# pnnl/nmrfit

Hardware: AMD Instinct MI355X
Metric: objective evals/sec (swarm x grid x peaks) (higher is better)
Workload: dtype f64

## Files before the change

### nmrfit_amd/csrc/objective_pair.h

```cpp
#pragma once
#include "objective_chunk.h"
#include "objective_finish.h"
#include "objective_launch.h"
#include "objective_lds.h"
#include "objective_prologue.h"
#include "swarm_prologue.h"

#include <type_traits>

namespace nmrfit {
namespace {

struct PairSide {
    PeakLor *lor;
    PeakFast *lorf;
    double2 *grec;
    PeakWin *win;
    double2 *seeds;
    double *shr;
    double *state;
    double *wsums;
    double base;
    bool rec_all;
};

template <bool FAST, bool FULL>
__device__ __forceinline__ void pair_model(const PairSide &s, const int P, const int lane, const double2 mm,
                                           const double (&wv)[kPointsPerLane], double (&acc)[kPointsPerLane])
{
    const double base = s.base;
    int k = 0;
    {
        const int kend0 = (P < kWave) ? P : kWave;
        if (kGroupSize <= kend0) {
            if constexpr (FAST)
                lorentz_group_fast<kGroupSize, true>(s.lorf, wv, acc, base);
            else
                lorentz_group<kGroupSize, true>(s.lor, wv, acc, base);
            k = kGroupSize;
        } else if (kend0 > 0) {
            if constexpr (FAST)
                lorentz_tail_fast<true>(kend0, s.lorf, wv, acc, base);
            else
                lorentz_tail<kGroupSize, true>(kend0, s.lor, wv, acc, base);
            k = kend0;
        } else {
#pragma unroll
            for (int q = 0; q < kPointsPerLane; ++q) acc[q] = base;
        }
    }
    for (int kb = 0; kb < P; kb += kWave) {
        const int kend = (P < kb + kWave) ? P : kb + kWave;
        bool h = false;
        if (kb + lane < P) {
            const PeakWin wn = s.win[kb + lane];
            h = (mm.y >= (double)wn.lo) && (mm.x <= (double)wn.hi);
        }
        unsigned long long hits = __ballot(h);
        if (kb != 0) k = kb;
        if constexpr (FAST) {
            for (; k + kGroupSize <= kend; k += kGroupSize) lorentz_group_fast<kGroupSize>(s.lorf + k, wv, acc);
            if (k < kend) lorentz_tail_fast(kend - k, s.lorf + k, wv, acc);
        } else {
            for (; k + kGroupSize <= kend; k += kGroupSize) lorentz_group<kGroupSize>(s.lor + k, wv, acc);
            if (k < kend) lorentz_tail<kGroupSize>(kend - k, s.lor + k, wv, acc);
        }
        if (kend - kb < kWave) hits &= (1ull << (kend - kb)) - 1ull;
        const bool rec = FULL && s.rec_all;
        for (unsigned long long m = rec ? hits : 0ull; m; m &= m - 1) {
            const int k1 = kb + __builtin_ctzll(m);
            gauss_add_rec(s.lor + k1, s.grec + k1, wv, acc);
        }
        for (unsigned long long m = rec ? 0ull : hits; m; m &= m - 1) gauss_add<true>(s.lor + kb + __builtin_ctzll(m), wv, acc);
    }
}

struct PairState {
    double zr, zi, bs;
};
__device__ __forceinline__ PairState pair_state(const PairSide &s, const int lane, const bool first, const int bidx)
{
    PairState st;
    if (first) {
        const double2 e = s.seeds[bidx];
        const double lr = s.shr[2 + lane], li = s.shr[2 + kWave + lane];
        st.zr = __builtin_fma(e.x, lr, -(e.y * li));
        st.zi = __builtin_fma(e.x, li, e.y * lr);
    } else {
        st.zr = s.state[lane];
        st.zi = s.state[kWave + lane];
    }
    st.bs = s.state[2 * kWave + lane];
    return st;
}

__device__ __forceinline__ void pair_epilogue(const PairSide &s, const int lane, const PairState &st, const bool last, const int slot,
                                              const double (&acc)[kPointsPerLane], const double (&uq)[kPointsPerLane],
                                              const double (&vq)[kPointsPerLane], const double (&tq)[kPointsPerLane])
{
    double zr = st.zr, zi = st.zi, bs = st.bs;
    const double rr = s.shr[0], ri = s.shr[1];
#pragma unroll
    for (int q = 0; q < kPointsPerLane; ++q) {
        const double vd = __builtin_fma(zr, uq[q], -(zi * vq[q]));
        const double e = tq[q] * (vd - acc[q]);
        bs = __builtin_fma(e, e, bs);
        const double nzr = __builtin_fma(zr, rr, -(zi * ri));
        zi = __builtin_fma(zr, ri, zi * rr);
        zr = nzr;
    }
    if (last) {
        const double cs = wave_sum(bs);
        bs = 0.0;
        if (lane == 0) s.wsums[slot] = cs;
    }
    s.state[lane] = zr;
    s.state[kWave + lane] = zi;
    s.state[2 * kWave + lane] = bs;
}

template <int WPB>
__device__ __forceinline__ void objective_pair_body(
    unsigned char *lds_raw, double *wsums2, const double *__restrict__ wc, const double *__restrict__ u,
    const double *__restrict__ v, const double *__restrict__ wt, const double2 *__restrict__ chunk_minmax,
    const double *__restrict__ X, int64_t S, int P, int64_t N, double w0, double wspan, int64_t seg_len, int blk_chunks,
    int seg_blocks, int n_blocks_i, double lane_step, double rec_devk, double *__restrict__ out,
    unsigned long long *__restrict__ clk, const PsoFused &upd)
{
    static_assert(WPB == kWavesPerBlock, "the pair layout is sized for four-wave workgroups");
    const int lane = threadIdx.x & (kWave - 1);
    const int wave = __builtin_amdgcn_readfirstlane((int)(threadIdx.x >> 6));
    const ObjectivePairLds at = objective_pair_lds_layout(P);
    int64_t part[kPairParticles] = {2 * (int64_t)blockIdx.x, 2 * (int64_t)blockIdx.x + 1};
    const bool hasB = part[1] < S;
    const int64_t D = 4 + 3 * (int64_t)P;
    const bool fused = upd.x_in != nullptr;
    const int rows = (upd.tail != 0u) ? 3 : 1;
    double *xrow[kPairParticles];
    PairSide side[kPairParticles];
    int *sflag[kPairParticles];
#pragma unroll
    for (int h = 0; h < kPairParticles; ++h) {
        side[h].lor = reinterpret_cast<PeakLor *>(lds_raw + ObjectivePairLds::lor) + (size_t)h * P;
        side[h].lorf = reinterpret_cast<PeakFast *>(lds_raw + at.lorf) + (size_t)h * P;
        side[h].grec = reinterpret_cast<double2 *>(lds_raw + at.grec) + (size_t)h * P;
        side[h].win = reinterpret_cast<PeakWin *>(lds_raw + at.win) + (size_t)h * P;
        side[h].seeds = reinterpret_cast<double2 *>(lds_raw + at.seeds) + ((size_t)h * WPB + wave) * kMaxBlocks;
        side[h].shr = reinterpret_cast<double *>(lds_raw + at.shr + (size_t)h * kSharedPrologueBytes);
        side[h].state = reinterpret_cast<double *>(lds_raw + at.state + (size_t)wave * kPairStateBytes) + (size_t)h * 3 * kWave;
        side[h].wsums = wsums2 + (size_t)h * kWsumsCount;
        sflag[h] = reinterpret_cast<int *>(side[h].shr + 2 + 2 * kWave);
        xrow[h] = reinterpret_cast<double *>(lds_raw + upd.xrow_off) + (size_t)h * rows * D;
    }
    f64x2 *const park = reinterpret_cast<f64x2 *>(lds_raw + at.park + (size_t)wave * kPairParkBytes);
    phase_stamp(clk, 0);
    if (clk && blockIdx.x == 0 && wave == 0 && lane == 0) {
        clk[0] = __builtin_amdgcn_s_memtime();
        clk[1] = __builtin_amdgcn_s_memrealtime();
    }
    if (fused) {
        const bool stopped = swarm_prologue<WPB>(upd, xrow[0], D, S, part[0], wave, true, true, wave, lane, side[0].wsums, clk);
        if (hasB) swarm_prologue<WPB>(upd, xrow[1], D, S, part[1], wave, true, true, wave, lane, side[1].wsums, clk);
        if (stopped) return;
    }
    const double invN = 1.0 / (double)N;
    double p1[kPairParticles] = {0.0, 0.0};
#pragma unroll
    for (int h = 0; h < kPairParticles; ++h) {
        if (h == 1 && !hasB) break;
        double p0, r, yoff;
        bool fast_bad = false, rec_bad = false;
        const StagePeakConstants<true, true> stage_peaks{p0, p1[h], r, yoff, P, lane, w0, wspan, side[h].lor, side[h].win, fast_bad,
                                                         side[h].lorf, lane_step, rec_devk, rec_bad, side[h].grec};
        const int turn = (wave + 2 * h) & (WPB - 1);
        if (fused)
            stage_peaks(xrow[h], turn, WPB);
        else
            stage_peaks(X + part[h] * D, turn, WPB);
        if (turn == WPB - 1) {
            double sr, si, tr, ti;
            sincos_fast((p1[h] * 64.0) * invN, &si, &sr);
            sincos_fast(p0 + (p1[h] * (double)lane) * invN, &ti, &tr);
            if (lane == 0) {
                side[h].shr[0] = sr;
                side[h].shr[1] = si;
            }
            side[h].shr[2 + lane] = tr;
            side[h].shr[2 + kWave + lane] = ti;
        }
        const int fl = (__ballot(fast_bad) != 0ull ? 1 : 0) | (__ballot(rec_bad) != 0ull ? 2 : 0);
        if (lane == 0) sflag[h][wave] = fl;
        side[h].base = wave_uniform((double)P * yoff);
    }
    __syncthreads();
    bool fast_all[kPairParticles] = {true, true};
#pragma unroll
    for (int h = 0; h < kPairParticles; ++h) {
        side[h].rec_all = false;
        if (h == 1 && !hasB) break;
        int all = 0;
#pragma unroll
        for (int w2 = 0; w2 < WPB; ++w2) all |= sflag[h][w2];
        fast_all[h] = !(all & 1);
        side[h].rec_all = !(all & 2);
    }
    phase_stamp(clk, 2);

    const int seg = wave;
    const int64_t j0 = (int64_t)seg * seg_len;
    const int64_t j1 = (j0 + seg_len < N) ? j0 + seg_len : N;
    const int64_t blk_len = (int64_t)blk_chunks * kChunk;
    const int64_t n_blocks = n_blocks_i;
    const int64_t b0 = (int64_t)seg * seg_blocks;
    const int64_t nb = (seg_blocks < n_blocks - b0) ? seg_blocks : n_blocks - b0;
#pragma unroll
    for (int h = 0; h < kPairParticles; ++h) {
        if (h == 1 && !hasB) break;
        if (lane < nb) {
            double er, ei;
            sincos_fast((p1[h] * (double)((b0 + lane) * blk_len)) * invN, &ei, &er);
            side[h].seeds[lane] = make_double2(er, ei);
        }
        side[h].state[2 * kWave + lane] = 0.0;
    }
    wave_lds_fence();
    const int blk0 = (int)b0;
    int cib = 0, bidx = 0;

    auto chunk = [&](const int64_t jb, const bool doA, const bool doB, auto fast_tag, auto full_tag) {
        constexpr bool kFastLoop = decltype(fast_tag)::value;
        constexpr bool full = decltype(full_tag)::value;
        const int64_t jl = jb + lane;
        double wv[kPointsPerLane], accA[kPointsPerLane], accB[kPointsPerLane];
        double uq[kPointsPerLane], vq[kPointsPerLane], tq[kPointsPerLane];
        if (full) {
            const global_pairs wp = lane_ptr(wc + jb, lane);
#pragma unroll
            for (int m = 0; m < kPointsPerLane / 2; ++m) {
                const f64x2 d = wp[m * kWave];
                wv[2 * m] = d.x;
                wv[2 * m + 1] = d.y;
            }
        } else {
#pragma unroll
            for (int q = 0; q < kPointsPerLane; ++q)
                wv[q] = (jl + q * kWave < j1) ? wc[jb + (q >> 1) * (2 * kWave) + 2 * lane + (q & 1)] : 0.0;
        }
        const double2 mm = global_table(chunk_minmax, jb / kChunk);
        if (doA) {
            pair_model<kFastLoop, full>(side[0], P, lane, mm, wv, accA);
#pragma unroll
            for (int m = 0; m < kPointsPerLane / 2; ++m) park[m * kWave + lane] = f64x2{accA[2 * m], accA[2 * m + 1]};
        }
        if (doB) pair_model<kFastLoop, full>(side[1], P, lane, mm, wv, accB);
        asm volatile("" ::: "memory");
        if (full) {
            const global_pairs up = lane_ptr(u + jb, lane), vp = lane_ptr(v + jb, lane), tp = lane_ptr(wt + jb, lane);
#pragma unroll
            for (int m = 0; m < kPointsPerLane / 2; ++m) {
                const f64x2 du = up[m * kWave], dv = vp[m * kWave], dt = tp[m * kWave];
                uq[2 * m] = du.x;
                uq[2 * m + 1] = du.y;
                vq[2 * m] = dv.x;
                vq[2 * m + 1] = dv.y;
                tq[2 * m] = dt.x;
                tq[2 * m + 1] = dt.y;
            }
        } else {
#pragma unroll
            for (int q = 0; q < kPointsPerLane; ++q) {
                const bool ok = jl + q * kWave < j1;
                const int64_t js = jb + (q >> 1) * (2 * kWave) + 2 * lane + (q & 1);
                uq[q] = ok ? u[js] : 0.0;
                vq[q] = ok ? v[js] : 0.0;
                tq[q] = ok ? wt[js] : 0.0;
            }
        }
        const bool first = cib == 0;
        const bool last = (cib + 1 == blk_chunks) || (jb + kChunk >= j1);
        if (doB) pair_epilogue(side[1], lane, pair_state(side[1], lane, first, bidx), last, blk0 + bidx, accB, uq, vq, tq);
        if (doA) {
            wave_lds_fence();
#pragma unroll
            for (int m = 0; m < kPointsPerLane / 2; ++m) {
                const f64x2 d = park[m * kWave + lane];
                accA[2 * m] = d.x;
                accA[2 * m + 1] = d.y;
            }
            pair_epilogue(side[0], lane, pair_state(side[0], lane, first, bidx), last, blk0 + bidx, accA, uq, vq, tq);
        }
        wave_lds_fence();
        ++cib;
        if (last) {
            cib = 0;
            ++bidx;
        }
    };
    auto chunk_loop = [&](const bool doA, const bool doB, auto fast_tag) {
        cib = 0;
        bidx = 0;
        int64_t jb = j0;
        for (; jb + kChunk <= j1; jb += kChunk) chunk(jb, doA, doB, fast_tag, std::true_type{});
        if (jb < j1) chunk(jb, doA, doB, fast_tag, std::false_type{});
    };
    if (fast_all[0] && fast_all[1]) {
        chunk_loop(true, hasB, std::true_type{});
    } else {
        if (fast_all[0])
            chunk_loop(true, false, std::true_type{});
        else
            chunk_loop(true, false, std::false_type{});
        if (hasB) {
            if (fast_all[1])
                chunk_loop(false, true, std::true_type{});
            else
                chunk_loop(false, true, std::false_type{});
        }
    }

    phase_stamp(clk, 3);
    if (clk && blockIdx.x == 0 && wave == 0 && lane == 0) {
        clk[2] = __builtin_amdgcn_s_memtime();
        clk[3] = __builtin_amdgcn_s_memrealtime();
    }
    __syncthreads();
#pragma unroll
    for (int h = 0; h < kPairParticles; ++h) {
        if (wave != h || (h == 1 && !hasB)) continue;
        double *wsums = side[h].wsums;
        if (lane == 0) {
            double t = 0.0;
            for (int64_t c = 0; c < n_blocks; ++c) t += wsums[c];
            const double f = sqrt(t / (double)N);
            out[part[h]] = f;
            wsums[2 * kMaxBlocks] = f;
        }
        wave_lds_fence();
        phase_stamp(clk, 4);
        const PersonalBest<false> personal_best{wsums, P, part[h], lds_raw, clk};
        personal_best(wsums[2 * kMaxBlocks]);
    }
}

template <int WPB = kWavesPerBlock>
__global__ __launch_bounds__(kWave *WPB, kMinWaves) void objective_kernel_pair(
    const double *__restrict__ wc, const double *__restrict__ u, const double *__restrict__ v,
    const double *__restrict__ wt, const double2 *__restrict__ chunk_minmax, const double *__restrict__ X, int64_t S,
    int P, int64_t N, double w0, double wspan, int64_t seg_len, int blk_chunks, int seg_blocks, int n_blocks,
    double lane_step, double rec_devk, double *__restrict__ out, unsigned long long *__restrict__ clk, const PsoFused upd)
{
    extern __shared__ __align__(16) unsigned char lds_raw[];
    __shared__ double wsums2[kPairParticles * kWsumsCount];
    if (threadIdx.x < kPairParticles) {
        const int h = threadIdx.x;
        double *wsums = wsums2 + h * kWsumsCount;
        const int64_t particle = 2 * (int64_t)blockIdx.x + h;
        const int64_t D = 4 + 3 * (int64_t)P;
        const bool pbest = upd.x_in != nullptr && upd.pbest != 0u;
        wsums[2 * kMaxBlocks + 1] = pbest ? 1.0 : 0.0;
        wsums[2 * kMaxBlocks + 2] = __longlong_as_double((long long)(uintptr_t)upd.p);
        wsums[2 * kMaxBlocks + 3] = __longlong_as_double((long long)S);
        wsums[2 * kMaxBlocks + 4] = __longlong_as_double((long long)(upd.xrow_off + (unsigned)h * (upd.tail != 0u ? 3u : 1u) * (unsigned)(D * sizeof(double))));
        if (pbest && particle < S) wsums[2 * kMaxBlocks + 5] = upd.p[S * D + particle];
        wsums[2 * kMaxBlocks + 7] = __longlong_as_double((pbest && upd.tail != 0u) ? (long long)upd.pflip : 0LL);
    }
    objective_pair_body<WPB>(lds_raw, wsums2, wc, u, v, wt, chunk_minmax, X, S, P, N, w0, wspan, seg_len, blk_chunks, seg_blocks,
                             n_blocks, lane_step, rec_devk, out, clk, upd);
}

}
}
```

Measured before the change: 5581 billion.

## Recompute pair LDS pointers on demand and steer scalar/vector register placement in pair kernel

Replaces the per-side struct of precomputed LDS pointers with a templated side that derives each pointer from the LDS base on demand. Adds empty inline-asm constraints that pin values to scalar or vector registers, and uses pointer cursors that advance per chunk instead of indexing from the chunk start. Also makes the A/B selection compile-time, computes the last-chunk flag without branches, loads the window test unconditionally with two ballots, and broadcasts the wave sum so every lane writes it. The aim is lower register pressure and less 64-bit address arithmetic in the hot loop. The catch is extra pointer recomputation and fragile compiler-steering tricks, and the unguarded window load can read past P.

After: 5622 billion (median of 6 runs). About the same (+0.7%).

```diff
diff --git a/nmrfit_amd/csrc/objective_pair.h b/nmrfit_amd/csrc/objective_pair.h
--- a/nmrfit_amd/csrc/objective_pair.h
+++ b/nmrfit_amd/csrc/objective_pair.h
@@ -11,38 +11,45 @@
 namespace nmrfit {
 namespace {
 
+template <int H>
 struct PairSide {
-    PeakLor *lor;
-    PeakFast *lorf;
-    double2 *grec;
-    PeakWin *win;
-    double2 *seeds;
-    double *shr;
-    double *state;
-    double *wsums;
+    unsigned char *lds;
+    double *wsums2;
+    int P, Prec, wave;
     double base;
-    bool rec_all;
+    int rec_all;
+    __device__ __forceinline__ PeakLor *lor() const { return reinterpret_cast<PeakLor *>(lds + ObjectivePairLds::lor) + (size_t)H * Prec; }
+    __device__ __forceinline__ PeakFast *lorf() const { return reinterpret_cast<PeakFast *>(lds + objective_pair_lds_layout(Prec).lorf) + (size_t)H * Prec; }
+    __device__ __forceinline__ double2 *grec() const { return reinterpret_cast<double2 *>(lds + objective_pair_lds_layout(Prec).grec) + (size_t)H * Prec; }
+    __device__ __forceinline__ PeakWin *win() const { return reinterpret_cast<PeakWin *>(lds + objective_pair_lds_layout(Prec).win) + (size_t)H * Prec; }
+    __device__ __forceinline__ double2 *seeds() const { return reinterpret_cast<double2 *>(lds + objective_pair_lds_layout(P).seeds) + ((size_t)H * kWavesPerBlock + wave) * kMaxBlocks; }
+    __device__ __forceinline__ double *shr() const { return reinterpret_cast<double *>(lds + objective_pair_lds_layout(P).shr + (size_t)H * kSharedPrologueBytes); }
+    __device__ __forceinline__ double *state() const { return reinterpret_cast<double *>(lds + objective_pair_lds_layout(P).state + (size_t)wave * kPairStateBytes) + (size_t)H * 3 * kWave; }
+    __device__ __forceinline__ double *wsums() const { return wsums2 + (size_t)H * kWsumsCount; }
+    __device__ __forceinline__ int *sflag() const { return reinterpret_cast<int *>(shr() + 2 + 2 * kWave); }
 };
 
-template <bool FAST, bool FULL>
-__device__ __forceinline__ void pair_model(const PairSide &s, const int P, const int lane, const double2 mm,
+template <bool FAST, bool FULL, int H>
+__device__ __forceinline__ void pair_model(const PairSide<H> &s, const int P, const int lane, const double2 mm,
                                            const double (&wv)[kPointsPerLane], double (&acc)[kPointsPerLane])
 {
     const double base = s.base;
+    PeakLor *const lor = s.lor();
+    PeakFast *const lorf = s.lorf();
     int k = 0;
     {
         const int kend0 = (P < kWave) ? P : kWave;
         if (kGroupSize <= kend0) {
             if constexpr (FAST)
-                lorentz_group_fast<kGroupSize, true>(s.lorf, wv, acc, base);
+                lorentz_group_fast<kGroupSize, true>(lorf, wv, acc, base);
             else
-                lorentz_group<kGroupSize, true>(s.lor, wv, acc, base);
+                lorentz_group<kGroupSize, true>(lor, wv, acc, base);
             k = kGroupSize;
         } else if (kend0 > 0) {
             if constexpr (FAST)
-                lorentz_tail_fast<true>(kend0, s.lorf, wv, acc, base);
+                lorentz_tail_fast<true>(kend0, lorf, wv, acc, base);
             else
-                lorentz_tail<kGroupSize, true>(kend0, s.lor, wv, acc, base);
+                lorentz_tail<kGroupSize, true>(kend0, lor, wv, acc, base);
             k = kend0;
         } else {
 #pragma unroll
@@ -51,55 +58,68 @@
     }
     for (int kb = 0; kb < P; kb += kWave) {
         const int kend = (P < kb + kWave) ? P : kb + kWave;
-        bool h = false;
-        if (kb + lane < P) {
-            const PeakWin wn = s.win[kb + lane];
-            h = (mm.y >= (double)wn.lo) && (mm.x <= (double)wn.hi);
-        }
-        unsigned long long hits = __ballot(h);
+        int kl = kb + lane;
+        asm volatile("" : "+v"(kl));
+        const PeakWin wn = s.win()[kl];
+        unsigned long long hits = __builtin_amdgcn_ballot_w64(mm.y >= (double)wn.lo) & __builtin_amdgcn_ballot_w64(mm.x <= (double)wn.hi);
         if (kb != 0) k = kb;
         if constexpr (FAST) {
-            for (; k + kGroupSize <= kend; k += kGroupSize) lorentz_group_fast<kGroupSize>(s.lorf + k, wv, acc);
-            if (k < kend) lorentz_tail_fast(kend - k, s.lorf + k, wv, acc);
+            for (; k + kGroupSize <= kend; k += kGroupSize) lorentz_group_fast<kGroupSize>(lorf + k, wv, acc);
+            if (k < kend) lorentz_tail_fast(kend - k, lorf + k, wv, acc);
         } else {
-            for (; k + kGroupSize <= kend; k += kGroupSize) lorentz_group<kGroupSize>(s.lor + k, wv, acc);
-            if (k < kend) lorentz_tail<kGroupSize>(kend - k, s.lor + k, wv, acc);
+            for (; k + kGroupSize <= kend; k += kGroupSize) lorentz_group<kGroupSize>(lor + k, wv, acc);
+            if (k < kend) lorentz_tail<kGroupSize>(kend - k, lor + k, wv, acc);
         }
         if (kend - kb < kWave) hits &= (1ull << (kend - kb)) - 1ull;
-        const bool rec = FULL && s.rec_all;
+        const bool rec = FULL && s.rec_all != 0;
         for (unsigned long long m = rec ? hits : 0ull; m; m &= m - 1) {
             const int k1 = kb + __builtin_ctzll(m);
-            gauss_add_rec(s.lor + k1, s.grec + k1, wv, acc);
-        }
-        for (unsigned long long m = rec ? 0ull : hits; m; m &= m - 1) gauss_add<true>(s.lor + kb + __builtin_ctzll(m), wv, acc);
-    }
-}
+            gauss_add_rec(lor + k1, s.grec() + k1, wv, acc);
+        }
+        for (unsigned long long m = rec ? 0ull : hits; m; m &= m - 1) gauss_add<true>(lor + kb + __builtin_ctzll(m), wv, acc);
+    }
+}
+
+struct PairCursor {
+    const double *w, *u, *v, *t;
+    const double2 *mm;
+    __device__ __forceinline__ void advance()
+    {
+        w += kChunk;
+        u += kChunk;
+        v += kChunk;
+        t += kChunk;
+        ++mm;
+    }
+};
 
 struct PairState {
     double zr, zi, bs;
 };
-__device__ __forceinline__ PairState pair_state(const PairSide &s, const int lane, const bool first, const int bidx)
+template <int H>
+__device__ __forceinline__ PairState pair_state(const PairSide<H> &s, const int lane, const bool first, const int bidx)
 {
     PairState st;
     if (first) {
-        const double2 e = s.seeds[bidx];
-        const double lr = s.shr[2 + lane], li = s.shr[2 + kWave + lane];
+        const double2 e = s.seeds()[bidx];
+        const double lr = s.shr()[2 + lane], li = s.shr()[2 + kWave + lane];
         st.zr = __builtin_fma(e.x, lr, -(e.y * li));
         st.zi = __builtin_fma(e.x, li, e.y * lr);
     } else {
-        st.zr = s.state[lane];
-        st.zi = s.state[kWave + lane];
-    }
-    st.bs = s.state[2 * kWave + lane];
+        st.zr = s.state()[lane];
+        st.zi = s.state()[kWave + lane];
+    }
+    st.bs = s.state()[2 * kWave + lane];
     return st;
 }
 
-__device__ __forceinline__ void pair_epilogue(const PairSide &s, const int lane, const PairState &st, const bool last, const int slot,
+template <int H>
+__device__ __forceinline__ void pair_epilogue(const PairSide<H> &s, const int lane, const PairState &st, const bool last, const int slot,
                                               const double (&acc)[kPointsPerLane], const double (&uq)[kPointsPerLane],
                                               const double (&vq)[kPointsPerLane], const double (&tq)[kPointsPerLane])
 {
     double zr = st.zr, zi = st.zi, bs = st.bs;
-    const double rr = s.shr[0], ri = s.shr[1];
+    const double rr = s.shr()[0], ri = s.shr()[1];
 #pragma unroll
     for (int q = 0; q < kPointsPerLane; ++q) {
         const double vd = __builtin_fma(zr, uq[q], -(zi * vq[q]));
@@ -111,12 +131,15 @@
     }
     if (last) {
         const double cs = wave_sum(bs);
+        int from0 = 0;
+        asm volatile("" : "+v"(from0));
+        const int cl = __builtin_amdgcn_ds_bpermute(from0, __double2loint(cs)), ch = __builtin_amdgcn_ds_bpermute(from0, __double2hiint(cs));
         bs = 0.0;
-        if (lane == 0) s.wsums[slot] = cs;
-    }
-    s.state[lane] = zr;
-    s.state[kWave + lane] = zi;
-    s.state[2 * kWave + lane] = bs;
+        s.wsums()[slot] = __hiloint2double(ch, cl);
+    }
+    s.state()[lane] = zr;
+    s.state()[kWave + lane] = zi;
+    s.state()[2 * kWave + lane] = bs;
 }
 
 template <int WPB>
@@ -130,48 +153,38 @@
     static_assert(WPB == kWavesPerBlock, "the pair layout is sized for four-wave workgroups");
     const int lane = threadIdx.x & (kWave - 1);
     const int wave = __builtin_amdgcn_readfirstlane((int)(threadIdx.x >> 6));
-    const ObjectivePairLds at = objective_pair_lds_layout(P);
     int64_t part[kPairParticles] = {2 * (int64_t)blockIdx.x, 2 * (int64_t)blockIdx.x + 1};
     const bool hasB = part[1] < S;
     const int64_t D = 4 + 3 * (int64_t)P;
     const bool fused = upd.x_in != nullptr;
     const int rows = (upd.tail != 0u) ? 3 : 1;
     double *xrow[kPairParticles];
-    PairSide side[kPairParticles];
-    int *sflag[kPairParticles];
-#pragma unroll
-    for (int h = 0; h < kPairParticles; ++h) {
-        side[h].lor = reinterpret_cast<PeakLor *>(lds_raw + ObjectivePairLds::lor) + (size_t)h * P;
-        side[h].lorf = reinterpret_cast<PeakFast *>(lds_raw + at.lorf) + (size_t)h * P;
-        side[h].grec = reinterpret_cast<double2 *>(lds_raw + at.grec) + (size_t)h * P;
-        side[h].win = reinterpret_cast<PeakWin *>(lds_raw + at.win) + (size_t)h * P;
-        side[h].seeds = reinterpret_cast<double2 *>(lds_raw + at.seeds) + ((size_t)h * WPB + wave) * kMaxBlocks;
-        side[h].shr = reinterpret_cast<double *>(lds_raw + at.shr + (size_t)h * kSharedPrologueBytes);
-        side[h].state = reinterpret_cast<double *>(lds_raw + at.state + (size_t)wave * kPairStateBytes) + (size_t)h * 3 * kWave;
-        side[h].wsums = wsums2 + (size_t)h * kWsumsCount;
-        sflag[h] = reinterpret_cast<int *>(side[h].shr + 2 + 2 * kWave);
-        xrow[h] = reinterpret_cast<double *>(lds_raw + upd.xrow_off) + (size_t)h * rows * D;
-    }
-    f64x2 *const park = reinterpret_cast<f64x2 *>(lds_raw + at.park + (size_t)wave * kPairParkBytes);
+#pragma unroll
+    for (int h = 0; h < kPairParticles; ++h) xrow[h] = reinterpret_cast<double *>(lds_raw + upd.xrow_off) + (size_t)h * rows * D;
+    PairSide<0> sideA{lds_raw, wsums2, P, P, wave, 0.0, 0};
+    PairSide<1> sideB{lds_raw, wsums2, P, P, wave, 0.0, 0};
+    f64x2 *const park = reinterpret_cast<f64x2 *>(lds_raw + objective_pair_lds_layout(P).park + (size_t)wave * kPairParkBytes);
     phase_stamp(clk, 0);
     if (clk && blockIdx.x == 0 && wave == 0 && lane == 0) {
         clk[0] = __builtin_amdgcn_s_memtime();
         clk[1] = __builtin_amdgcn_s_memrealtime();
     }
     if (fused) {
-        const bool stopped = swarm_prologue<WPB>(upd, xrow[0], D, S, part[0], wave, true, true, wave, lane, side[0].wsums, clk);
-        if (hasB) swarm_prologue<WPB>(upd, xrow[1], D, S, part[1], wave, true, true, wave, lane, side[1].wsums, clk);
+        const bool stopped = swarm_prologue<WPB>(upd, xrow[0], D, S, part[0], wave, true, true, wave, lane, sideA.wsums(), clk);
+        if (hasB) swarm_prologue<WPB>(upd, xrow[1], D, S, part[1], wave, true, true, wave, lane, sideB.wsums(), clk);
         if (stopped) return;
     }
     const double invN = 1.0 / (double)N;
     double p1[kPairParticles] = {0.0, 0.0};
-#pragma unroll
-    for (int h = 0; h < kPairParticles; ++h) {
-        if (h == 1 && !hasB) break;
+    auto stage_side = [&](auto &sd, const int h) {
         double p0, r, yoff;
         bool fast_bad = false, rec_bad = false;
-        const StagePeakConstants<true, true> stage_peaks{p0, p1[h], r, yoff, P, lane, w0, wspan, side[h].lor, side[h].win, fast_bad,
-                                                         side[h].lorf, lane_step, rec_devk, rec_bad, side[h].grec};
+        PeakLor *lor = sd.lor();
+        PeakWin *win = sd.win();
+        PeakFast *lorf = sd.lorf();
+        double2 *grec = sd.grec();
+        const StagePeakConstants<true, true> stage_peaks{p0, p1[h], r, yoff, P, lane, w0, wspan, lor, win, fast_bad,
+                                                         lorf, lane_step, rec_devk, rec_bad, grec};
         const int turn = (wave + 2 * h) & (WPB - 1);
         if (fused)
             stage_peaks(xrow[h], turn, WPB);
@@ -182,28 +195,31 @@
             sincos_fast((p1[h] * 64.0) * invN, &si, &sr);
             sincos_fast(p0 + (p1[h] * (double)lane) * invN, &ti, &tr);
             if (lane == 0) {
-                side[h].shr[0] = sr;
-                side[h].shr[1] = si;
+                sd.shr()[0] = sr;
+                sd.shr()[1] = si;
             }
-            side[h].shr[2 + lane] = tr;
-            side[h].shr[2 + kWave + lane] = ti;
+            sd.shr()[2 + lane] = tr;
+            sd.shr()[2 + kWave + lane] = ti;
         }
         const int fl = (__ballot(fast_bad) != 0ull ? 1 : 0) | (__ballot(rec_bad) != 0ull ? 2 : 0);
-        if (lane == 0) sflag[h][wave] = fl;
-        side[h].base = wave_uniform((double)P * yoff);
-    }
+        if (lane == 0) sd.sflag()[wave] = fl;
+        sd.base = wave_uniform((double)P * yoff);
+    };
+    stage_side(sideA, 0);
+    if (hasB) stage_side(sideB, 1);
     __syncthreads();
     bool fast_all[kPairParticles] = {true, true};
-#pragma unroll
-    for (int h = 0; h < kPairParticles; ++h) {
-        side[h].rec_all = false;
-        if (h == 1 && !hasB) break;
+    auto flags_of = [&](auto &sd, const int h) {
         int all = 0;
 #pragma unroll
-        for (int w2 = 0; w2 < WPB; ++w2) all |= sflag[h][w2];
+        for (int w2 = 0; w2 < WPB; ++w2) all |= sd.sflag()[w2];
+        all = __builtin_amdgcn_readfirstlane(all);
         fast_all[h] = !(all & 1);
-        side[h].rec_all = !(all & 2);
-    }
+        sd.rec_all = (all & 2) ? 0 : 1;
+    };
+    flags_of(sideA, 0);
+    if (hasB) flags_of(sideB, 1);
+    const int recs_all = __builtin_amdgcn_readfirstlane(sideA.rec_all | (sideB.rec_all << 1));
     phase_stamp(clk, 2);
 
     const int seg = wave;
@@ -213,28 +229,48 @@
     const int64_t n_blocks = n_blocks_i;
     const int64_t b0 = (int64_t)seg * seg_blocks;
     const int64_t nb = (seg_blocks < n_blocks - b0) ? seg_blocks : n_blocks - b0;
-#pragma unroll
-    for (int h = 0; h < kPairParticles; ++h) {
-        if (h == 1 && !hasB) break;
+    auto seed_side = [&](auto &sd, const int h) {
         if (lane < nb) {
             double er, ei;
             sincos_fast((p1[h] * (double)((b0 + lane) * blk_len)) * invN, &ei, &er);
-            side[h].seeds[lane] = make_double2(er, ei);
-        }
-        side[h].state[2 * kWave + lane] = 0.0;
-    }
+            sd.seeds()[lane] = make_double2(er, ei);
+        }
+        sd.state()[2 * kWave + lane] = 0.0;
+    };
+    seed_side(sideA, 0);
+    if (hasB) seed_side(sideB, 1);
     wave_lds_fence();
     const int blk0 = (int)b0;
+    const int nfull = (j1 > j0) ? (int)((j1 - j0) / kChunk) : 0;
+    const bool ragged = j0 + (int64_t)nfull * kChunk < j1;
+    const unsigned last_left = ragged ? 0u : 1u;
     int cib = 0, bidx = 0;
-
-    auto chunk = [&](const int64_t jb, const bool doA, const bool doB, auto fast_tag, auto full_tag) {
+    unsigned loff = (unsigned)lane * 16u;
+
+    auto chunk = [&](const PairCursor &g, const int64_t jb, const int left, auto a_tag, auto b_tag, auto fast_tag, auto full_tag) {
+        constexpr bool doA = decltype(a_tag)::value;
+        constexpr bool doB = decltype(b_tag)::value;
         constexpr bool kFastLoop = decltype(fast_tag)::value;
         constexpr bool full = decltype(full_tag)::value;
         const int64_t jl = jb + lane;
         double wv[kPointsPerLane], accA[kPointsPerLane], accB[kPointsPerLane];
         double uq[kPointsPerLane], vq[kPointsPerLane], tq[kPointsPerLane];
+        int Pc = P;
+        asm volatile("" : "+s"(Pc));
+        PairSide<0> sa = sideA;
+        PairSide<1> sb = sideB;
+        sa.Prec = Pc;
+        sb.Prec = Pc;
+        int recs = recs_all;
+        asm volatile("" : "+s"(recs));
+        sa.rec_all = recs & 1;
+        sb.rec_all = recs & 2;
+        asm volatile("" : "+v"(loff));
+        auto lane_pairs = [&](const double *uniform_base) {
+            return reinterpret_cast<global_pairs>(reinterpret_cast<const char __attribute__((address_space(1))) *>((uintptr_t)uniform_base) + (size_t)loff);
+        };
         if (full) {
-            const global_pairs wp = lane_ptr(wc + jb, lane);
+            const global_pairs wp = lane_pairs(g.w);
 #pragma unroll
             for (int m = 0; m < kPointsPerLane / 2; ++m) {
                 const f64x2 d = wp[m * kWave];
@@ -244,18 +280,20 @@
         } else {
 #pragma unroll
             for (int q = 0; q < kPointsPerLane; ++q)
-                wv[q] = (jl + q * kWave < j1) ? wc[jb + (q >> 1) * (2 * kWave) + 2 * lane + (q & 1)] : 0.0;
-        }
-        const double2 mm = global_table(chunk_minmax, jb / kChunk);
-        if (doA) {
-            pair_model<kFastLoop, full>(side[0], P, lane, mm, wv, accA);
+                wv[q] = (jl + q * kWave < j1) ? g.w[(q >> 1) * (2 * kWave) + 2 * lane + (q & 1)] : 0.0;
+        }
+        const f64x2 mmv = *reinterpret_cast<const f64x2 __attribute__((address_space(4))) *>((uintptr_t)g.mm);
+        const double2 mm = make_double2(mmv.x, mmv.y);
+        if constexpr (doA) {
+            pair_model<kFastLoop, full>(sa, Pc, lane, mm, wv, accA);
 #pragma unroll
             for (int m = 0; m < kPointsPerLane / 2; ++m) park[m * kWave + lane] = f64x2{accA[2 * m], accA[2 * m + 1]};
         }
-        if (doB) pair_model<kFastLoop, full>(side[1], P, lane, mm, wv, accB);
+        if constexpr (doB) pair_model<kFastLoop, full>(sb, Pc, lane, mm, wv, accB);
         asm volatile("" ::: "memory");
+        asm volatile("" : "+v"(loff));
         if (full) {
-            const global_pairs up = lane_ptr(u + jb, lane), vp = lane_ptr(v + jb, lane), tp = lane_ptr(wt + jb, lane);
+            const global_pairs up = lane_pairs(g.u), vp = lane_pairs(g.v), tp = lane_pairs(g.t);
 #pragma unroll
             for (int m = 0; m < kPointsPerLane / 2; ++m) {
                 const f64x2 du = up[m * kWave], dv = vp[m * kWave], dt = tp[m * kWave];
@@ -270,16 +308,18 @@
 #pragma unroll
             for (int q = 0; q < kPointsPerLane; ++q) {
                 const bool ok = jl + q * kWave < j1;
-                const int64_t js = jb + (q >> 1) * (2 * kWave) + 2 * lane + (q & 1);
-                uq[q] = ok ? u[js] : 0.0;
-                vq[q] = ok ? v[js] : 0.0;
-                tq[q] = ok ? wt[js] : 0.0;
+                const int js = (q >> 1) * (2 * kWave) + 2 * lane + (q & 1);
+                uq[q] = ok ? g.u[js] : 0.0;
+                vq[q] = ok ? g.v[js] : 0.0;
+                tq[q] = ok ? g.t[js] : 0.0;
             }
         }
-        const bool first = cib == 0;
-        const bool last = (cib + 1 == blk_chunks) || (jb + kChunk >= j1);
-        if (doB) pair_epilogue(side[1], lane, pair_state(side[1], lane, first, bidx), last, blk0 + bidx, accB, uq, vq, tq);
-        if (doA) {
+        int cibA = cib, cibB = cib;
+        const unsigned to_end = full ? min((unsigned)(cib + 1) ^ (unsigned)blk_chunks, (unsigned)left ^ last_left) : 0u;
+        const int last = (int)((to_end - 1u) >> 31);
+        asm volatile("" : "+s"(cibB));
+        if constexpr (doB) pair_epilogue(sb, lane, pair_state(sb, lane, cibB == 0, bidx), last != 0, blk0 + bidx, accB, uq, vq, tq);
+        if constexpr (doA) {
             wave_lds_fence();
 #pragma unroll
             for (int m = 0; m < kPointsPerLane / 2; ++m) {
@@ -287,58 +327,61 @@
                 accA[2 * m] = d.x;
                 accA[2 * m + 1] = d.y;
             }
-            pair_epilogue(side[0], lane, pair_state(side[0], lane, first, bidx), last, blk0 + bidx, accA, uq, vq, tq);
+            asm volatile("" : "+s"(cibA));
+            pair_epilogue(sa, lane, pair_state(sa, lane, cibA == 0, bidx), last != 0, blk0 + bidx, accA, uq, vq, tq);
         }
         wave_lds_fence();
-        ++cib;
-        if (last) {
-            cib = 0;
-            ++bidx;
-        }
+        cib = last ? 0 : cib + 1;
+        bidx += last;
     };
-    auto chunk_loop = [&](const bool doA, const bool doB, auto fast_tag) {
+    auto chunk_loop = [&](auto a_tag, auto b_tag, auto fast_tag) {
         cib = 0;
         bidx = 0;
-        int64_t jb = j0;
-        for (; jb + kChunk <= j1; jb += kChunk) chunk(jb, doA, doB, fast_tag, std::true_type{});
-        if (jb < j1) chunk(jb, doA, doB, fast_tag, std::false_type{});
+        PairCursor g{wc + j0, u + j0, v + j0, wt + j0, chunk_minmax + j0 / kChunk};
+        for (int left = nfull; left > 0; --left, g.advance()) chunk(g, 0, left, a_tag, b_tag, fast_tag, std::true_type{});
+        if (ragged) chunk(g, j0 + (int64_t)nfull * kChunk, 0, a_tag, b_tag, fast_tag, std::false_type{});
     };
-    if (fast_all[0] && fast_all[1]) {
-        chunk_loop(true, hasB, std::true_type{});
+    constexpr std::true_type yes{};
+    constexpr std::false_type no{};
+    if (fast_all[0] && fast_all[1] && hasB) {
+        chunk_loop(yes, yes, yes);
     } else {
         if (fast_all[0])
-            chunk_loop(true, false, std::true_type{});
+            chunk_loop(yes, no, yes);
         else
-            chunk_loop(true, false, std::false_type{});
+            chunk_loop(yes, no, no);
         if (hasB) {
             if (fast_all[1])
-                chunk_loop(false, true, std::true_type{});
+                chunk_loop(no, yes, yes);
             else
-                chunk_loop(false, true, std::false_type{});
-        }
-    }
-
+                chunk_loop(no, yes, no);
+        }
+    }
+
+    unsigned park_lane = (unsigned)(uintptr_t)(park + lane);
+    asm volatile("" : "+v"(park_lane));
+    const unsigned park_lane0 = (unsigned)(uintptr_t)(reinterpret_cast<f64x2 *>(lds_raw + objective_pair_lds_layout(P).park) + lane);
+    const int wave_end = __builtin_amdgcn_readfirstlane((int)((park_lane - park_lane0) / (unsigned)kPairParkBytes));
     phase_stamp(clk, 3);
-    if (clk && blockIdx.x == 0 && wave == 0 && lane == 0) {
+    if (clk && blockIdx.x == 0 && wave_end == 0 && lane == 0) {
         clk[2] = __builtin_amdgcn_s_memtime();
         clk[3] = __builtin_amdgcn_s_memrealtime();
     }
     __syncthreads();
-#pragma unroll
-    for (int h = 0; h < kPairParticles; ++h) {
-        if (wave != h || (h == 1 && !hasB)) continue;
-        double *wsums = side[h].wsums;
+    if (wave_end == 0 || (wave_end == 1 && hasB)) {
+        double *wsums = wsums2 + (size_t)wave_end * kWsumsCount;
+        const int64_t particle = part[0] + wave_end;
         if (lane == 0) {
             double t = 0.0;
             for (int64_t c = 0; c < n_blocks; ++c) t += wsums[c];
             const double f = sqrt(t / (double)N);
-            out[part[h]] = f;
+            out[particle] = f;
             wsums[2 * kMaxBlocks] = f;
         }
         wave_lds_fence();
         phase_stamp(clk, 4);
-        const PersonalBest<false> personal_best{wsums, P, part[h], lds_raw, clk};
-        personal_best(wsums[2 * kMaxBlocks]);
+        const PersonalBest<false> personal_best{wsums, P, particle, lds_raw, clk};
+        [[clang::always_inline]] personal_best(wsums[2 * kMaxBlocks]);
     }
 }
 
```
